# lgalke/aae-recommender

Hardware: AMD Instinct MI355X
Metric: train docs/sec at |items|=100k h=200 (higher is better)
Workload: dtype f32; 1 GPU; C3 PubMed-scale synthetic Bags: |items|=100000, hidden=200, code=50, fp32, batch=100 docs/GPU/step, full partial_fit (ae+disc+gen, 4 Adam) inside the AdversarialAutoEncoder.fit epoch loop (permutation batches of a corpus resident in HBM); n_items=100000, n_hidden=200, n_code=50, batch_per_gpu=100, global_batch=100, cond_inc=0, rng=device, parallelism=dp1

## Files before the change

### aae-recommender_amd/csrc/aae_abi.hip

```cpp
#include <hip/hip_runtime.h>
#include <hip/hip_ext.h>
#include <math.h>
#include <stdio.h>
#include <stdlib.h>
#include <string.h>

#include <algorithm>
#include <string>
#include <vector>

#include "../../include/aaerec_hip.h"
#include "gemm_f32.h"
#include "kernels.h"
#include "dec_fused.h"
#include "dec_fused_bf16.h"
#include "dec_crit_x3.h"
#include "rank_x3.h"
#include "rank_long.h"
#include "rank_full.h"
#include "cooc.h"
#include "spgemm.h"
#include "sptrans.h"
#include "mutinfo.h"
#include "popular.h"
// ... 106 lines not shown
        }
        m->x16_ok = m->use_chain4 && m->FXi[P_W2] != nullptr;
        if (m->x16_ok) each_chain16x3(limit(m->x16_ok, kX16Lds));
        m->force_unfused = cfg->unfused_decoder == 1;
        if (m->fused_ok) {
            each_dec_fused(kDecFused, limit(m->fused_ok, maxlds));
            if (m->bf16) each_dec_fused_bf16(kDecFused, limit(m->fused_ok, maxlds));
            if (!raise_lds_limit(tile_bucket_kernel, maxlds - 2048)) m->fused_ok = false;
            m->bucket_wide_ok = raise_lds_limit(tile_bucket_wide_kernel, maxlds - 16384);
            {
                hipFuncAttributes fa;
                static bool told = false;
                if (m->bucket_wide_ok && !told && hipFuncGetAttributes(&fa, reinterpret_cast<const void*>(tile_bucket_wide_kernel)) == hipSuccess && fa.numRegs < 121) {
                    told = true;
                    fprintf(stderr, "aaerec: tile_bucket_wide_kernel allocates %d vector registers, not the 128 it claims to keep its CU to itself (buckets.h)\n", fa.numRegs);
                }
                (void)hipGetLastError();
            }
        }
    }
    m->late_enabled = !m->opt.no_late_join;
    m->early_enabled = true;
    m->early_any = m->opt.early_any;
    m->rank_ok = m->fused_ok && m->use_chain4 && !m->vae && !m->opt.no_rank_fused;
    m->vae_rank_ok = m->vae && m->fused_ok && m->use_chain4 && !m->opt.no_rank_fused;
    if (m->vae_rank_ok) each_chain4_vae(limit(m->vae_rank_ok, kCSlots * kCR * kCL * sizeof(float)));
    bool& rank_ok = m->vae ? m->vae_rank_ok : m->rank_ok;
    if (rank_ok) each_rank_x3([&](RankKernel k, int nb) { rank_ok = rank_ok && raise_lds_limit(k, rank_x3_lds_bytes(nb)); });
    if (rank_ok) each_rank_x3v2([&](RankKernel k, int nb) { rank_ok = rank_ok && raise_lds_limit(k, rank_x3v2_lds_bytes(nb)); });
    m->w1_big_lds = raise_lds_limit(w1_item_update_kernel, sizeof(int) * w1_items_lds_words(16384));
    (void)hipGetLastError();
    m->grad_scale = 1.f;
    m->rng_row0 = 0; m->rng_global = 0;
    m->Gt = m->G.p;
    m->split_ok = false; m->opt_pending = false; m->side = nullptr; m->ev_crit = m->ev_opt = nullptr;
    m->split_wgs = std::max(1, (m->n_cu * 5) / 8);
    m->pf_armed = m->pf_built = m->pf_pending = false; m->pf_step = -1; m->hstep = 0; m->flushed_hstep = -1; m->ev_head = m->ev_pf = nullptr;
    bool side_ok = false;
    if (cfg->grad_mode == AAE_GRAD_FUSED) {
        int lo = 0, hi = 0;
        const unsigned evflags = hipEventDisableTiming | hipEventDisableSystemFence;
        side_ok = hipDeviceGetStreamPriorityRange(&lo, &hi) == hipSuccess &&
                  hipStreamCreateWithPriority(&m->side, hipStreamNonBlocking, lo) == hipSuccess &&
                  hipEventCreateWithFlags(&m->ev_crit, evflags) == hipSuccess &&
                  hipEventCreateWithFlags(&m->ev_opt, evflags) == hipSuccess &&
                  hipEventCreateWithFlags(&m->ev_head, evflags) == hipSuccess &&
                  hipEventCreateWithFlags(&m->ev_pf, evflags) == hipSuccess &&
                  hipEventCreateWithFlags(&m->ev_bk, evflags) == hipSuccess &&
                  hipEventCreateWithFlags(&m->ev_end, evflags) == hipSuccess;
        if (!side_ok) {
            if (m->side) (void)hipStreamDestroy(m->side);
            m->side = nullptr;
        }
        (void)hipGetLastError();
    }
    if (side_ok && m->fused_ok && m->bf16 && m->split_wgs > 0 &&
        (size_t)((m->N + kBU - 1) / kBU) * kBU * bf_stride(4) <= (size_t)m->R * m->ldn) {
        m->split_ok = true;
        for (int mode : {kDecCrit, kDecOpt}) each_dec_fused_bf16(mode, limit(m->split_ok, maxlds));
        (void)hipGetLastError();
    }
    if (side_ok && m->fused_ok && m->split_wgs > 0 && 
        (size_t)((m->N + kTI - 1) / kTI) * kTI * (size_t)std::min(m->R, 16 * kMB) * sizeof(float) < (size_t)0x7FFFFFF0u) {
        bool ok = true;
        for (int mode : {kDecCrit, kDecOpt, kDecOptAcc}) each_dec_fused(mode, limit(ok, maxlds));
        each_dec_opt_blocks(limit(ok, maxlds));
        if (!m->bf16) m->split_ok = ok;
        m->x3_ok = ok;
        each_dec_crit_x3(false, limit(m->x3_ok, maxlds));
        each_dec_opt_blocks_x3(limit(m->x3_ok, maxlds));
        each_dec_opt_x3(false, limit(m->x3_ok, maxlds));
        (void)hipGetLastError();
        if (m->bf16) {
            m->bf16_x3 = m->x3_ok && ok;
            if (!m->bf16_x3) m->x3_ok = false;
            else m->split_ok = true;
            m->bf16_one = m->bf16_x3;
            each_dec_crit_x3(true, limit(m->bf16_one, maxlds));
            each_dec_opt_x3(true, limit(m->bf16_one, maxlds));
            (void)hipGetLastError();
        }
        if (m->x3_ok) {
            const int ntiles = (m->N + 31) / 32;
            const double t_tile = (3.3 + 0.0131 * m->h) * (m->bf16_one ? 0.87 : 1.0);
            int w = (int)(ntiles * t_tile / (m->bf16_one ? 165.0 : 82.0) / 8.0 + 0.5) * 8;
            w = std::max(w, std::min(ntiles, m->bf16_one ? 48 : 64));
            const int cap = m->late_enabled ? m->n_cu * 15 / 32 : m->n_cu * 9 / 16;
            m->split_wgs = std::max(1, std::min(w, cap));
        }
    }
    hipStream_t s = S(stream);
    hipError_t e = hipMemsetAsync(arena_dev, 0, need, s);
    if (e != hipSuccess) { delete m; return fail(AAE_EHIP, std::string("hipMemsetAsync: ") + hipGetErrorString(e)); }
    struct { Ten* t; int col; } ones[] = {{&m->eh1, m->h}, {&m->eh2, m->h}, {&m->zc, m->cp}, {&m->dh1, m->h},
                                           {&m->dh2, m->h}, {&m->zin, m->c}, {&m->xh1, m->h}, {&m->xh2, m->h}};
    for (auto& o : ones)
        hipLaunchKernelGGL(fill_col_kernel, dim3(((int)o.t->rows + 255) / 256), dim3(256), 0, s, o.t->p, (int)o.t->ld,
                           (int)o.t->rows, o.col, 1.0f);
    OptScalars hs[4]; memset(hs, 0, sizeof(hs));
    for (int i = 0; i < 4; ++i) {
        hs[i].t = 0; hs[i].is_sgd = cfg->optimizer == AAE_OPT_SGD;
        hs[i].lr = (i == O_ENC || i == O_DEC) ? (double)cfg->gen_lr : (double)cfg->reg_lr;
        hs[i].neg_step_size = 0.f; hs[i].bc2_sqrt = 1.f; hs[i].inv_bc2_sqrt = 1.f;
    }
    e = hipMemcpyAsync(m->sc, hs, sizeof(hs), hipMemcpyHostToDevice, s);
    if (e == hipSuccess) e = hipStreamSynchronize(s);
    if (e != hipSuccess) { delete m; return fail(AAE_EHIP, std::string("init: ") + hipGetErrorString(e)); }
    *out = m;
    return AAE_OK;
}

#ifdef W1_TS
int aae_debug_w1_ts(unsigned long long* out, int n) {
    return (int)hipMemcpyFromSymbol(out, HIP_SYMBOL(aae::w1_ts), sizeof(unsigned long long) * (size_t)n);
}
#endif
int aae_destroy(aae_handle h) {
    if (!h) return AAE_OK;
    if (h->side) {
        (void)hipStreamSynchronize(h->side);
        (void)hipStreamDestroy(h->side);
    }
    if (h->dp_scratch) (void)hipFree(h->dp_scratch);
    if (h->cnt_host) (void)hipHostFree(h->cnt_host);
    for (hipEvent_t e : {h->ev_crit, h->ev_opt, h->ev_head, h->ev_pf, h->ev_bk, h->ev_end}) if (e) (void)hipEventDestroy(e);
    if (h->prof_ev) {
        for (int k = 0; k < AAE_K_N; ++k)
            for (auto& pr : h->prof_ev[k]) { (void)hipEventDestroy(pr.first); (void)hipEventDestroy(pr.second); }
        delete[] h->prof_ev;
    }
    delete h;
    return AAE_OK;
}


int aae_profile_enable(aae_handle h, int on) {
    if (!h) return fail(AAE_EINVAL, "handle is NULL");
    if (on && !h->prof_ev) h->prof_ev = new std::vector<std::pair<hipEvent_t, hipEvent_t>>[AAE_K_N];
    h->prof_on = on != 0;
    h->prof_mask = on == 1 ? ~0u : ((unsigned)on >> 1);
    return AAE_OK;
}

int aae_profile_read(aae_handle h, int kernel_id, double* total_ms, int64_t* launches) {
    if (!h || !total_ms || !launches) return fail(AAE_EINVAL, "NULL argument");
    if (kernel_id < 0 || kernel_id >= AAE_K_N) return fail(AAE_EINVAL, "bad kernel id");
    *total_ms = 0.0; *launches = 0;
    if (!h->prof_ev) return AAE_OK;
    auto& v = h->prof_ev[kernel_id];
    for (size_t i = 0; i < h->prof_used[kernel_id]; ++i) {
        HIPCHK(hipEventSynchronize(v[i].second));
        float ms = 0.f;
        HIPCHK(hipEventElapsedTime(&ms, v[i].first, v[i].second));
        *total_ms += ms; *launches += 1;
    }
    h->prof_used[kernel_id] = 0;
    return AAE_OK;
}

int aae_prefetch_batch(aae_handle h, const aae_batch* next) {
    if (!h || !next) return fail(AAE_EINVAL, "NULL argument");
    if (!next->indptr_dev || !next->indices_dev || !next->values_dev) return fail(AAE_EINVAL, "batch pointers are NULL");
    if (next->n_rows < 1 || next->n_rows > h->R) return fail(AAE_EINVAL, "batch n_rows outside [1, max_batch]");
    if (next->nnz_bound > h->cfg.max_nnz) return fail(AAE_EINVAL, "batch nnz_bound > max_nnz");
    if (next->generation == 0) { h->pf_armed = false; return AAE_OK; }
    h->pf_batch = *next;
    h->pf_armed = true;
    return AAE_OK;
}

// ... 117 lines not shown
```

### aae-recommender_amd/csrc/abi_output_layer.h

```cpp
#pragma once

namespace {

struct DecLaunch {
    DecFusedArgs fa;
    int nblk, Bb;
    int ntiles, grid;
    bool win;
    size_t fused_lds;
    bool want_ts, ts_obk;
};
unsigned long long* dec_ts_dev = nullptr;

DecFusedArgs fill_dec_args(const aae_model* m, int B, int nblk, float gscale) {
    DecFusedArgs fa;
    fa.dh2 = m->dh2.p; fa.ldh = m->ldh;
    fa.V3a = m->P[P_V3].p; fa.M = m->M[0][P_V3].p; fa.V = m->V[0][P_V3].p; fa.ldv = m->ldh;
    fa.gradV3 = m->cfg.grad_mode == AAE_GRAD_EXPORT ? m->Gr[P_V3].p : nullptr;
    fa.N = m->N; fa.B = B; fa.h = m->h; fa.gscale = gscale;
    fa.te.start = m->tstart; fa.te.eb = m->teb; fa.te.en = m->ten; fa.te.ev = m->tev;
    fa.slabs = m->slabs.p; fa.slab_stride = (size_t)(nblk > 1 ? B : std::min(m->R, 16 * kMB)) * m->ldh; fa.ld_slab = m->ldh;
    fa.partials = m->bce_partials; fa.sc = m->sc + O_DEC;
    fa.erow0 = 0; fa.acc = nullptr; fa.nblk = 1; fa.Bb = B;
    fa.one_term = m->bf16_x3 ? 1 : 0; fa.dbg_skip = m->opt.dec_skip;
// ... 37 lines not shown
        for (int k = 0; k < 5; ++k) {
            fprintf(stderr, "[dec_fused_bf16 arrivals at barrier %d, us after the unit's start]", k);
            for (int w = 0; w < 16; ++w) fprintf(stderr, " %.2f", ((double)t[16 + 16 * k + w] - (double)t[0]) * 0.01);
            fprintf(stderr, "\n");
        }
    fprintf(stderr, "[dec_fused tile 5] S0=%.2f GEMM1+BCE0=%.2f entries=%.2f GEMM2+GEMM3=%.2f S5=%.2f | tile=%.2f us, %.0f shader clocks -> %.2f GHz\n",
            (t[1] - t[0]) * 0.01, (t[2] - t[1]) * 0.01, (t[3] - t[2]) * 0.01, (t[4] - t[3]) * 0.01,
            (t[6] - t[4]) * 0.01, (t[6] - t[0]) * 0.01, (double)(t[9] - t[8]),
            (double)(t[9] - t[8]) / ((t[6] - t[0]) * 10.0));
    if (out_bf16(m)) fprintf(stderr, "[dec_fused_bf16 S0] barrier A=%.2f work=%.2f barrier B=%.2f us\n", (t[14] - t[0]) * 0.01, (t[15] - t[14]) * 0.01, (t[1] - t[15]) * 0.01);
    fprintf(stderr, "[dec_fused wg 0] prologue=%.2f loop=%.2f (%llu tiles, %.2f each) epilogue=%.2f us\n",
            (t[11] - t[10]) * 0.01, (t[7] - t[11]) * 0.01, t[13], (t[7] - t[11]) * 0.01 / (double)(t[13] ? t[13] : 1),
            (t[12] - t[7]) * 0.01);
    return AAE_OK;
}

int launch_output_critical(aae_model* m, const DecLaunch& L, bool late, int grid, hipStream_t s) {
    DecFusedArgs b = L.fa;
    b.nblk = L.nblk; b.Bb = L.Bb;
    if (late) { b.dh2_snap = m->dh2s.p; b.sc_snap = m->sc_snap; }
    hipEvent_t start = nullptr, stop = m->ev_crit;
    (void)prof_pair(m, AAE_K_DEC_CRIT, &start, &stop);
    const int nb = m->fused_nb;
    DecKernel kernel; int threads = kNT; uint32_t lds = (uint32_t)L.fused_lds;
    if (out_bf16(m)) { kernel = pick_dec_fused_bf16(nb, kDecCrit); threads = kBT; }
    else if (m->x3_ok) {
        const bool ts = b.ts && !m->bf16_one && nb == 13;
        kernel = pick_dec_crit_x3(nb, ts, m->bf16_one, L.win && !ts);
        lds = (uint32_t)dec_crit_x3_lds_bytes(nb);
    } else kernel = pick_dec_fused(nb, kDecCrit, L.win);
    if (!kernel) return no_kernel("dec_fused (critical launch)");
    hipExtLaunchKernelGGL(kernel, dim3(grid), dim3(threads), lds, s, start, stop, 0, b);
    LAUNCHCHK("dec_fused (critical launch)");
    HIPCHK(hipStreamWaitEvent(m->side, stop, 0));
    return AAE_OK;
}

int launch_deferred(aae_model* m, DecKernel kernel, const char* what, int grid, int threads, uint32_t lds, const DecFusedArgs& b) {
    if (!kernel) return no_kernel(what);
    hipEvent_t start = nullptr, stop = nullptr;
    (void)prof_pair(m, AAE_K_DEC_OPT, &start, &stop);
    hipExtLaunchKernelGGL(kernel, dim3(grid), dim3(threads), lds, m->side, start, stop, 0, b);
    LAUNCHCHK(what);
    return AAE_OK;
}

int launch_output_deferred(aae_model* m, const DecLaunch& L, bool late, bool* late_launched) {
    const DecFusedArgs& fa = L.fa;
    const int nblk = L.nblk, Bb = L.Bb, ntiles = L.ntiles, nb = m->fused_nb, B = fa.B;
    const int g2 = std::min(ntiles, std::min(m->split_wgs, m->n_cu));
    DecFusedArgs b = fa;
    b.nblk = nblk; b.Bb = Bb;
    if (nblk > 1 && !out_bf16(m) && m->x3_ok && m->dh2f.p) {
        hipLaunchKernelGGL(dh2_frag_kernel, dim3((B + kXCH - 1) / kXCH, m->fused_nb), dim3(128), 0, m->side, m->dh2.p, m->ldh, B,
                           reinterpret_cast<u32x4_t*>(m->dh2f.p), b.one_term);
        b.acc = m->dh2f.p;
        const int wg_cap = ntiles >= 4096 ? m->n_cu * 7 / 8 : m->n_cu * 3 / 4;
        const int by_tiles = ntiles < 384 ? std::max(32, std::min(m->n_cu / 2, ntiles / 3))
                                          : std::max(m->n_cu / 2, std::min(wg_cap, (int)(ntiles / 16.3 / 8.0 + 0.5) * 8));
        const int g3 = std::max(1, std::min(by_tiles, std::min(ntiles, m->n_cu)));
        const int rounds = (ntiles + g3 * kXBT - 1) / (g3 * kXBT);
        b.tpp = g3 * rounds;
        const uint32_t lds3 = (uint32_t)dec_opt_blocks_x3_lds_bytes();
        const bool ts = L.ts_obk && nb == 13;
        TRY(launch_deferred(m, pick_dec_opt_blocks_x3(nb, ts, L.win && !ts), "dec_opt_blocks_x3", g3, kNT, lds3, b));
        return ts ? print_dec_timeline(m, true, false, m->side) : AAE_OK;
    }
    if (nblk > 1 && !out_bf16(m) && ntiles <= kOBT * m->n_cu && dec_opt_blocks_lds_bytes(Bb) <= 160 * 1024) {
        const int g3 = std::max(std::min(g2, ntiles), (ntiles + kOBT - 1) / kOBT);
        return launch_deferred(m, pick_dec_opt_blocks(nb), "dec_opt_blocks", g3, kNT, (uint32_t)dec_opt_blocks_lds_bytes(Bb), b);
    }
    for (int r = 0; r < nblk; ++r) {
        b = fa;
        const int r0 = r * Bb;
        b.B = std::min(Bb, B - r0); b.erow0 = r0;
        b.dh2 = fa.dh2 + (size_t)r0 * m->ldh;
        b.slabs = fa.slabs + (size_t)r0 * m->ldh;
        b.partials = fa.partials + (size_t)r * L.grid;
        b.Gt = fa.Gt + (size_t)r * ntiles * Bb * kTI;
        if (nblk > 1) { b.acc = m->Gacc.p; b.gradV3 = r == nblk - 1 ? nullptr : m->Gacc.p; }
        const char* what = "dec_fused (optimiser launch)";
        if (out_bf16(m)) TRY(launch_deferred(m, pick_dec_fused_bf16(nb, kDecOpt), what, g2, kBT, (uint32_t)L.fused_lds, b));
        else if (nblk == 1 && m->x3_ok) {
            const uint32_t lds_nat = (uint32_t)dec_opt_x3_lds_bytes();
            const uint32_t lds3 = m->bf16_one ? std::max(lds_nat, 150u * 1024u) : lds_nat;
            if (late) { b.dh2 = m->dh2s.p; b.sc = m->sc_snap; *late_launched = true; }
            TRY(launch_deferred(m, pick_dec_opt_x3(nb, m->bf16_one, L.win), what, g2, kNT, lds3, b));
        } else TRY(launch_deferred(m, pick_dec_fused(nb, r == 0 ? kDecOpt : kDecOptAcc, L.win), what, g2, kNT, (uint32_t)L.fused_lds, b));
    }
    return AAE_OK;
}

int output_layer_split(aae_model* m, const DecLaunch& L, int* n_loss_partials, int* crit_slabs, hipStream_t s) {
    if (m->opt_pending) TRY(join_deferred(m, s));
    const int nblk = L.nblk;
    const bool late = m->late_enabled && nblk == 1 && m->x3_ok && !out_bf16(m) && !L.want_ts &&
                      m->dh2s.p && m->sc_snap && L.fa.B <= m->dh2s.rows && L.grid >= L.fa.B;
    const int wgs = nblk > 1 ? std::max(1, m->n_cu / nblk) : L.grid;
    const int crit_grid = nblk > 1 ? wgs * nblk : L.grid;
    *n_loss_partials = crit_grid;
    *crit_slabs = wgs;
    TRY(launch_output_critical(m, L, late, crit_grid, s));
    bool late_launched = false;
    TRY(launch_output_deferred(m, L, late, &late_launched));
    TRY(side_done(m, m->ev_opt));
    m->opt_pending = true;
    m->late_ok = late_launched;
    m->last_out_split = true; m->side_ordered = true;
    if (m->only_output_layer && m->pf_armed && m->mark2 && m->lazy) TRY(launch_prefetch(m, false));
    return AAE_OK;
}

int launch_output_single(aae_model* m, const DecLaunch& L, hipStream_t s) {
    m->last_out_split = false; m->side_ordered = false;
    ProfScope ps(m, AAE_K_DEC_FUSED, s);
    const DecKernel kernel = m->bf16 ? pick_dec_fused_bf16(m->fused_nb, kDecFused) : pick_dec_fused(m->fused_nb, kDecFused, L.win);
    if (!kernel) return no_kernel("dec_fused");
    const size_t lds = m->bf16 ? dec_fused_bf16_lds_bytes(m->fused_nb) : L.fused_lds;
    hipLaunchKernelGGL(kernel, dim3(L.grid), dim3(m->bf16 ? kBT : kNT), lds, s, L.fa);
    return AAE_OK;
}

int reduce_slabs(aae_model* m, const DecLaunch& L, int crit_slabs, int n_loss_partials, const DropSpec& d2, const float** part_out, hipStream_t s) {
    const int B = L.fa.B, N = m->N, h = m->h;
    const size_t slab_stride = L.fa.slab_stride;
    float* part = m->slabs.p + (size_t)304 * slab_stride;
    *part_out = part;
    const size_t n4 = (size_t)B * m->ldh / 4;
    auto sum_slabs = [&](const float* src, int n, float* dst, size_t dst_stride, int ny, bool loss) {
        hipLaunchKernelGGL(slab_partial_kernel, dim3((unsigned)((n4 + 255) / 256), ny), dim3(256), 0, s, src, n, slab_stride, n4, dst, dst_stride,
                           loss ? m->bce_partials : (const float*)nullptr, loss ? n_loss_partials : 0, loss ? 1.0f / ((float)B * (float)N) : 0.f, m->losses, 0);
    };
    if (m->only_output_layer && crit_slabs <= 64) {
        sum_slabs(m->slabs.p, crit_slabs, m->da2.p, 0, 1, true);
        LAUNCHCHK("slabs -> da2");
        return AAE_OK;
    }
    sum_slabs(m->slabs.p, crit_slabs, part, slab_stride, 16, true);
    if (m->only_output_layer) {
        sum_slabs(part, 16, m->da2.p, 0, 1, false);
        LAUNCHCHK("slab_partial -> da2");
    } else if (!m->use_chain) {
        hipLaunchKernelGGL(slab_reduce_actbwd_kernel, dim3(grid1d((size_t)B * h, 64)), dim3(64), 0, s, part, 16,
                           slab_stride, B, h, m->ldh, m->dh2.p, m->ldh, m->gb0.p, m->cfg.activation, d2,
                           m->cfg.seed, m->step_ctr);
        LAUNCHCHK("slab_reduce");
    }
    return AAE_OK;
}

int output_layer_fused(aae_model* m, int B, float gscale, const DropSpec& d2, const float** chain_part, size_t* chain_stride, hipStream_t s) {
    if (m->bk_pending) {
        HIPCHK(hipStreamWaitEvent(s, m->ev_bk, 0));
        m->bk_pending = false;
    }
    if (!m->buckets_valid) TRY(build_tile_buckets(m, s));
    DecLaunch L;
    L.nblk = m->have_batch ? row_blocks(m) : 1; L.Bb = (B + L.nblk - 1) / L.nblk;
    L.ntiles = (m->N + kTI - 1) / kTI; L.grid = std::min(L.ntiles, m->n_cu);
    L.win = x3_big_span(m->N, m->ldh);
    L.fused_lds = out_bf16(m) ? dec_fused_bf16_lds_bytes(m->fused_nb) : dec_fused_lds_bytes(L.Bb, m->h);
    L.fa = fill_dec_args(m, B, L.nblk, gscale);
    L.want_ts = m->opt.dec_ts[0] != 0;
    if (L.want_ts) {
        if (!dec_ts_dev && hipMalloc(&dec_ts_dev, 128 * sizeof(unsigned long long)) != hipSuccess) return fail(AAE_EHIP, "ts alloc");
        L.fa.ts = dec_ts_dev;
    }
// ... 144 lines not shown
```

### aae-recommender_amd/csrc/dec_crit_x3.h

```cpp
#pragma once
#include "dec_fused_bf16.h"

namespace aae {

typedef short s16x4_t __attribute__((ext_vector_type(4)));

__device__ __forceinline__ void split3_pair(float a, float b, unsigned& p1, unsigned& p2, unsigned& p3, bool one) {
    x3_split_pair(a, b, p1, p2, p3);
    if (one) { p2 = 0u; p3 = 0u; }
}
__device__ __forceinline__ f32x4 mfma_x3(const bf16x8 (&a)[3], const bf16x8 (&b)[3], f32x4 c) { return x3_mfma(a, b, c); }
template <bool ONE>
__device__ __forceinline__ f32x4 mfma_xt(const bf16x8 (&a)[3], const bf16x8 (&b)[3], f32x4 c) {
    if constexpr (ONE) return __builtin_amdgcn_mfma_f32_16x16x32_bf16(a[0], b[0], c, 0, 0, 0);
    else return x3_mfma(a, b, c);
}

__host__ __device__ constexpr int x3_stride(int kc) { return 16 * kc + 8; }
__device__ __forceinline__ bf16x8 x3_frag(const unsigned* img, int row, int S, int kc, int fk) {
    return __builtin_bit_cast(bf16x8, *reinterpret_cast<const u32x4_t*>(img + row * S + 16 * kc + 4 * fk));
}
constexpr int kXRS = 33;
constexpr int kXT = 32;

// ... 285 lines not shown
            const int lz = lane + oz, q = (lz >> 2) & 3, p = lz & 3;
            const unsigned* base = v3K + (8 * fkz + q) * S1 + 8 * cb + 2 * p;
#pragma unroll
            for (int t = 0; t < NT; ++t) {
                const s16x4_t lo = __builtin_amdgcn_ds_read_tr16_b64_v4i16(
                    (s16x4_t __attribute__((address_space(3)))*)(base + t * (kTI * S1)));
                const s16x4_t hi = __builtin_amdgcn_ds_read_tr16_b64_v4i16(
                    (s16x4_t __attribute__((address_space(3)))*)(base + t * (kTI * S1) + 4 * S1));
                typedef short s16x8_t __attribute__((ext_vector_type(8)));
                const s16x8_t v = {lo[0], lo[1], lo[2], lo[3], hi[0], hi[1], hi[2], hi[3]};
                vt[t] = __builtin_bit_cast(bf16x8, v);
            }
        };
        auto gemm3 = [&](auto Q0, auto Q1) {
#pragma unroll
            for (int q = decltype(Q0)::value; q < decltype(Q1)::value; ++q) {
                if (BAL && (q < q_lo || q >= q_hi)) continue;
                bf16x8 ga[3];
#pragma unroll
                for (int t = 0; t < NT; ++t) ga[t] = x3_frag(gK + t * (kGR * S3), 16 * q + frz, S3, 0, fkz);
                acc3[q] = mfma_xt<ONE>(ga, vt, acc3[q]);
            }
        };
        typedef std::integral_constant<int, 0> Q_0;
        typedef std::integral_constant<int, kMB> Q_E;
        constexpr int NJ = (kGR * (kTI / 2) + kNT - 1) / kNT;
        stamp(0);

        stamp(14);
        stamp(1);
        if (kCritG1Pf) {
            if (g1) { if (nks == NKS) gemm1_pf(std::integral_constant<int, NKS>()); else gemm1_pf(std::integral_constant<int, (NKS > 1 ? NKS - 1 : 1)>()); }
        } else if (g1) gemm1();
        load_span(min(tile + stride, ntiles - 1), vreg);
        lds_barrier();
        stamp(2);
        lprod = 1.f;
#pragma unroll
        for (int j = 0; j < NJ; ++j) bce(64 * wave + kNT * j);
        loss += log_pos(lprod);
        if (own) read_vt();
        lds_barrier();
        stamp(3);
        if (own) gemm3(Q_0(), Q_E());
        __builtin_amdgcn_sched_barrier(0);
        stage(tile + stride);
        stamp(4);
        __builtin_amdgcn_sched_barrier(0);
        lds_barrier();
        __builtin_amdgcn_sched_barrier(0);
        stamp(5);
        stamp(6);
    }
    if (TS && a.ts && blockIdx.x == 0 && tid == 0) a.ts[7] = wall_clock64();

    float* slab = slabs_blk + (size_t)wgi * a.slab_stride;
    if (own) {
#pragma unroll
        for (int q = 0; q < kMB; ++q) {
            const int rb = q * 16 + fk * 4, cc = cb * 16 + fr;
#pragma unroll
            for (int r = 0; r < 4; ++r)
                if (q >= q_lo && q < q_hi && rb + r < B && cc < a.ld_slab) slab[(size_t)(rb + r) * a.ld_slab + cc] = acc3[q][r];
        }
    }
    loss = wave_sum(loss);
    __syncthreads();
    if (lane == 0) red[wave] = loss;
    __syncthreads();
    if (tid == 0) {
        float s = 0.f;
        for (int w = 0; w < kNW; ++w) s += red[w];
        a.partials[blockIdx.x] = s;
        if (TS && a.ts && blockIdx.x == 0) { a.ts[12] = wall_clock64(); a.ts[13] = (unsigned long long)iter; }
    }
}

}

namespace aae {

constexpr int kXGS = 20;

inline size_t dec_opt_x3_lds_bytes() { return sizeof(float) * ((size_t)3 * 128 * kXGS + (size_t)kTI * kSO + 64); }

template <int NB, bool ONE = false, bool WIN = false>
__global__ __launch_bounds__(kNT) void dec_opt_x3_kernel(DecFusedArgs a) {
    const bool one = ONE || a.one_term != 0;
    constexpr int NT = ONE ? 1 : 3;
    constexpr int KR = 4;
    static_assert(NB <= 13, "column blocks 10..12 are the ones split over two waves");
    extern __shared__ __attribute__((aligned(16))) float lds[];
    unsigned* gB = reinterpret_cast<unsigned*>(lds);
    float* os = reinterpret_cast<float*>(gB + 3 * 128 * kXGS);
    const int tid = threadIdx.x, lane = tid & 63;
    const int wave = __builtin_amdgcn_readfirstlane(tid >> 6);
    const int fr = lane & 15, fk = lane >> 4;
    const int B = a.B, ldv = a.ldv, N = a.N;
    const int ntiles = (N + kTI - 1) / kTI;
    const int f4_per_row = ldv / 4, tile_f4 = kTI * f4_per_row;
    constexpr int NV = 2;
    const OptScalars sc = *a.sc;
    const bool do_adam = a.gradV3 == nullptr;
    typedef unsigned int fu32x4 __attribute__((ext_vector_type(4)));
    if (a.dbg_skip & 0x10000) return;
    if (a.dbg_skip & 0x20000) {
        const unsigned long long t0 = wall_clock64();
        while (wall_clock64() - t0 < 13500ull) __builtin_amdgcn_s_sleep(32);
        return;
    }

    for (int i = tid; i < 3 * 128 * kXGS; i += kNT) gB[i] = 0u;

    int cb, nb_lo, nb_hi;
    if (wave < 10) { cb = wave; nb_lo = 0; nb_hi = 2; }
    else { cb = 10 + ((wave - 10) >> 1); nb_lo = (wave - 10) & 1; nb_hi = nb_lo + 1; }
    const bool live = cb < NB;
    cb = min(cb, NB - 1);
    bf16x8 dB[KR][3];
    {
        const int c = min(16 * cb + fr, a.ldh - 1);
#pragma unroll
        for (int kc = 0; kc < KR; ++kc) {
            float x[8];
#pragma unroll
            for (int j = 0; j < 8; ++j) {
                const int b = 32 * kc + 8 * fk + j;
                x[j] = (b < B && 16 * cb + fr < a.ldh) ? a.dh2[(size_t)b * a.ldh + c] : 0.f;
            }
            unsigned p[3][4];
#pragma unroll
            for (int q = 0; q < 4; ++q) split3_pair(x[2 * q], x[2 * q + 1], p[0][q], p[1][q], p[2][q], one);
#pragma unroll
            for (int t = 0; t < NT; ++t) {
                const u32x4_t v = {p[t][0], p[t][1], p[t][2], p[t][3]};
                dB[kc][t] = __builtin_bit_cast(bf16x8, v);
            }
        }
    }

    const unsigned lane_off = (unsigned)tid * 16u;
    const unsigned tile_bytes = (unsigned)(kTI * ldv) * 4u;
    X3WindowT<WIN> win(N, ldv, tile_bytes);
    const float* gbase = a.gradV3 ? a.gradV3 : a.V3a;
    __amdgpu_buffer_rsrc_t rP = win.desc(a.V3a), rM = win.desc(a.M), rV = win.desc(a.V), rG = win.desc(gbase);
    const int g_f4 = B * (kTI / 4);
    const unsigned gbytes = (unsigned)min((size_t)0x7FFFFFF0u, (size_t)ntiles * g_f4 * 16);
    const __amdgpu_buffer_rsrc_t rGt = __builtin_amdgcn_make_buffer_rsrc(a.Gt, 0, gbytes, 0x00020000);
    auto ld4 = [&](const __amdgpu_buffer_rsrc_t& r, int tile, int j) {
        const unsigned vo = tid + kNT * j < tile_f4 ? lane_off + (unsigned)(kNT * 16 * j) : 0x80000000u;
        return __builtin_bit_cast(float4, __builtin_amdgcn_raw_buffer_load_b128(r, vo, win.so(tile), 2));
    };
    auto ldg = [&](int tile) {
        return __builtin_bit_cast(float4, __builtin_amdgcn_raw_buffer_load_b128(rGt, tid < g_f4 ? lane_off : 0x80000000u, (unsigned)tile * (unsigned)g_f4 * 16u, 2));
    };
    int s_rc[NV];
#pragma unroll
    for (int j = 0; j < NV; ++j) {
        const int fc = min(tid + kNT * j, tile_f4 - 1), row = fc / f4_per_row;
        s_rc[j] = row * 64 + (fc - row * f4_per_row);
    }
    float4 p_cur[NV], p_nxt[NV], mreg[NV], sreg[NV], g_nxt;
    int tile = blockIdx.x;
    const int stride = gridDim.x;
    if (tile < ntiles) {
#pragma unroll
        for (int j = 0; j < NV; ++j) p_nxt[j] = ld4(rP, tile, j);
        g_nxt = ldg(tile);
    }
    __syncthreads();

    for (; tile < ntiles; tile += stride) {
        const int i0 = tile * kTI;
        if (win.moves(tile)) { rP = win.desc(a.V3a); rM = win.desc(a.M); rV = win.desc(a.V); rG = win.desc(gbase); }
        int oz;
        asm volatile("v_mov_b32 %0, 0" : "=v"(oz));
        const int lz = lane + oz;
        lds_barrier();
        if (tid < g_f4) {
            unsigned q0[3], q1[3];
            split3_pair(g_nxt.x, g_nxt.y, q0[0], q0[1], q0[2], one);
            split3_pair(g_nxt.z, g_nxt.w, q1[0], q1[1], q1[2], one);
            unsigned* d = gB + (tid >> 3) * kXGS + (tid & 7) * 2;
#pragma unroll
            for (int t = 0; t < NT; ++t) *reinterpret_cast<uint2*>(d + t * (128 * kXGS)) = make_uint2(q0[t], q1[t]);
        }
#pragma unroll
        for (int j = 0; j < NV; ++j) p_cur[j] = p_nxt[j];
        g_nxt = ldg(min(tile + stride, ntiles - 1));
#pragma unroll
        for (int j = 0; j < NV; ++j) p_nxt[j] = ld4(rP, min(tile + stride, ntiles - 1), j);
#pragma unroll
        for (int j = 0; j < NV; ++j) { mreg[j] = ld4(rM, tile, j); sreg[j] = ld4(rV, tile, j); }
        lds_barrier();

        if (live) {
            const int tq = (lz >> 2) & 3, tp = lz & 3, g = lz >> 4;
            for (int nb2 = nb_lo; nb2 < nb_hi; ++nb2) {
                f32x4 c = (f32x4){0.f, 0.f, 0.f, 0.f};
                const unsigned* base = gB + (8 * g + tq) * kXGS + 8 * nb2 + 2 * tp;
#pragma unroll
                for (int kc = 0; kc < KR; ++kc) {
                    bf16x8 ga[3];
#pragma unroll
                    for (int t = 0; t < NT; ++t) {
                        const unsigned* pb = base + t * (128 * kXGS) + 32 * kc * kXGS;
                        const s16x4_t lo = __builtin_amdgcn_ds_read_tr16_b64_v4i16((s16x4_t __attribute__((address_space(3)))*)(pb));
                        const s16x4_t hi = __builtin_amdgcn_ds_read_tr16_b64_v4i16((s16x4_t __attribute__((address_space(3)))*)(pb + 4 * kXGS));
                        typedef short s16x8_t __attribute__((ext_vector_type(8)));
                        const s16x8_t v = {lo[0], lo[1], lo[2], lo[3], hi[0], hi[1], hi[2], hi[3]};
                        ga[t] = __builtin_bit_cast(bf16x8, v);
                    }
                    c = mfma_xt<ONE>(ga, dB[kc], c);
                }
#pragma unroll
                for (int r = 0; r < 4; ++r) os[(16 * nb2 + 4 * fk + r) * kSO + 16 * cb + fr] = c[r];
            }
        }
        lds_barrier();

#pragma unroll
        for (int j = 0; j < NV; ++j) {
            const bool valid = tid + kNT * j < tile_f4 && i0 + (s_rc[j] >> 6) < N;
            const float4 g = *reinterpret_cast<const float4*>(os + (s_rc[j] >> 6) * kSO + (s_rc[j] & 63) * 4);
            const unsigned so = win.so(tile);
            const unsigned vo = valid ? lane_off + (unsigned)(kNT * 16 * j) : 0x80000000u;
            float4 p = p_cur[j], mm = mreg[j], vv = sreg[j];
            adam_update(p.x, mm.x, vv.x, g.x, sc); adam_update(p.y, mm.y, vv.y, g.y, sc);
            adam_update(p.z, mm.z, vv.z, g.z, sc); adam_update(p.w, mm.w, vv.w, g.w, sc);
            const float4 out = do_adam ? p : g;
            const unsigned vo2 = (do_adam && !sc.is_sgd) ? vo : 0x80000000u;
            __builtin_amdgcn_raw_buffer_store_b128(__builtin_bit_cast(fu32x4, out), do_adam ? rP : rG, vo, so, 2);
            __builtin_amdgcn_raw_buffer_store_b128(__builtin_bit_cast(fu32x4, mm), rM, vo2, so, 2);
            __builtin_amdgcn_raw_buffer_store_b128(__builtin_bit_cast(fu32x4, vv), rV, vo2, so, 2);
        }
    }
}


constexpr int kXBT = 6;
constexpr int kXCH = 64;
constexpr int kXRowTab = 768;
constexpr int kXRing = 6;

__device__ __forceinline__ void glds16(const void* gsrc, unsigned lds_dst) {
    unsigned keep;
    asm volatile("s_mov_b32 %0, m0\n\ts_mov_b32 m0, %2\n\ts_nop 0\n\tglobal_load_lds_dwordx4 %1, off nt\n\ts_mov_b32 m0, %0"
                 : "=&s"(keep) : "v"(gsrc), "s"(lds_dst) : "memory");
}

inline size_t dec_opt_blocks_x3_lds_bytes() { return sizeof(float) * std::max((size_t)2 * 3 * 2 * kXCH * 8 + (size_t)kXRing * kXCH * kTI + 256 + 9 * kXRowTab, (size_t)kXBT * kTI * kSO); }

__global__ __launch_bounds__(128) void dh2_frag_kernel(const float* __restrict__ dh2, int ldh, int B, u32x4_t* __restrict__ out, int one_term) {
    const bool one = one_term != 0;
    const int ch = blockIdx.x, cb = blockIdx.y, nb = gridDim.y;
    const int kc = threadIdx.x >> 6, lane = threadIdx.x & 63, fr = lane & 15, fk = lane >> 4;
    const int c = 16 * cb + fr;
    float x[8];
#pragma unroll
    for (int j = 0; j < 8; ++j) {
        const int b = kXCH * ch + 32 * kc + 8 * fk + j;
        x[j] = (b < B && c < ldh) ? dh2[(size_t)b * ldh + c] : 0.f;
    }
    unsigned p[3][4];
#pragma unroll
    for (int q = 0; q < 4; ++q) split3_pair(x[2 * q], x[2 * q + 1], p[0][q], p[1][q], p[2][q], one);
#pragma unroll
    for (int t = 0; t < 3; ++t) {
        const u32x4_t v = {p[t][0], p[t][1], p[t][2], p[t][3]};
        out[((((size_t)ch * nb + cb) * (kXCH / 32) + kc) * 3 + t) * 64 + lane] = v;
    }
}

template <int NB, bool TS = false, bool WIN = false>
__global__ __launch_bounds__(kNT) void dec_opt_blocks_x3_kernel(DecFusedArgs a) {
    const bool one = a.one_term != 0;
    constexpr int KR = kXCH / 32;
    constexpr int IMG = 2 * kXCH * 8;
    auto slot_of = [](int r) { return (r & ~12) | ((r & 4) << 1) | ((r & 8) >> 1); };
    static_assert(NB <= kNW, "one column block per wave");
    extern __shared__ __attribute__((aligned(16))) float lds[];
    unsigned* gB = reinterpret_cast<unsigned*>(lds);
    float* ring = lds + 2 * 3 * IMG;
    unsigned* rowtab = reinterpret_cast<unsigned*>(ring + kXRing * kXCH * kTI + 256);
    float* os = lds;
    const int tid = threadIdx.x, lane = tid & 63;
    const int wave = __builtin_amdgcn_readfirstlane(tid >> 6);
    const int fr = lane & 15, fk = lane >> 4;
    const int ldv = a.ldv, N = a.N, B = a.B;
    const int ntiles = (N + kTI - 1) / kTI;
    const int f4_per_row = ldv / 4, tile_f4 = kTI * f4_per_row;
    constexpr int NV = 2;
    const OptScalars sc = *a.sc;
    typedef unsigned int fu32x4 __attribute__((ext_vector_type(4)));
    const int G = max(a.tpp, 1);
    const int nch = (B + kXCH - 1) / kXCH;
    const int cb = min(wave, NB - 1);

    const unsigned lane_off = (unsigned)tid * 16u;
    const unsigned tile_bytes = (unsigned)(kTI * ldv) * 4u;
    X3WindowT<WIN> win(N, ldv, tile_bytes);
    __amdgpu_buffer_rsrc_t rP = win.desc(a.V3a), rM = win.desc(a.M), rV = win.desc(a.V);
    auto ld4 = [&](const __amdgpu_buffer_rsrc_t& r, int tile, int j) {
        return __builtin_bit_cast(float4, __builtin_amdgcn_raw_buffer_load_b128(r, lane_off + (unsigned)(kNT * 16 * j), win.so(tile), 2));
    };
    constexpr int NM = NB + 1;
    constexpr int NL = (kNW - NM) * 64, NS = (kXCH * 8 + NL - 1) / NL;
    static_assert(NM < kNW, "no spare wave left");
    static_assert(kXCH * 8 * 2 == kNT, "one float4 of a slot per thread of the lower half");
    const bool mult = wave < NM;
    const int nb_lo = wave == NB ? 1 : 0, nb_hi = wave == NB - 1 ? 1 : 2;
    const int lt = tid - NM * 64;
// ... 197 lines not shown
```

Before: 432,600 docs/s.

## Prefetch next tile's Adam state interleaved with MFMA steps in dec_opt_x3

The x3 decoder optimiser kernel now prefetches the next tile's M and V moments along with P and the gradient. The individual prefetch loads are spread across the MFMA k-steps with scheduling barriers, so memory latency overlaps the GEMM instead of stalling before it. The third bf16 term of the decoder fragments moves from registers to LDS to reduce register pressure, and the Adam update is inlined with hardcoded beta constants. The split-workgroup heuristic constants are also retuned. Risks: more LDS per block, and the inlined update assumes beta1=0.9 and beta2=0.999.

After: 438,500 docs/s (median of 6 runs). 1.01x the previous value.

```diff
diff --git a/aae-recommender_amd/csrc/aae_abi.hip b/aae-recommender_amd/csrc/aae_abi.hip
--- a/aae-recommender_amd/csrc/aae_abi.hip
+++ b/aae-recommender_amd/csrc/aae_abi.hip
@@ -212,10 +212,10 @@
         }
         if (m->x3_ok) {
             const int ntiles = (m->N + 31) / 32;
-            const double t_tile = (3.3 + 0.0131 * m->h) * (m->bf16_one ? 0.87 : 1.0);
-            int w = (int)(ntiles * t_tile / (m->bf16_one ? 165.0 : 82.0) / 8.0 + 0.5) * 8;
-            w = std::max(w, std::min(ntiles, m->bf16_one ? 48 : 64));
-            const int cap = m->late_enabled ? m->n_cu * 15 / 32 : m->n_cu * 9 / 16;
+            const double t_tile = (2.2 + 0.0096 * m->h) * (m->bf16_one ? 0.98 : 1.0);
+            int w = (int)(ntiles * t_tile / (m->bf16_one ? 127.0 : 57.0) / 8.0 + 0.5) * 8;
+            w = std::max(w, std::min(ntiles, m->bf16_one ? 40 : 64));
+            const int cap = m->late_enabled ? m->n_cu * 7 / 16 : m->n_cu * 9 / 16;
             m->split_wgs = std::max(1, std::min(w, cap));
         }
     }
diff --git a/aae-recommender_amd/csrc/abi_output_layer.h b/aae-recommender_amd/csrc/abi_output_layer.h
--- a/aae-recommender_amd/csrc/abi_output_layer.h
+++ b/aae-recommender_amd/csrc/abi_output_layer.h
@@ -143,7 +143,7 @@
         const char* what = "dec_fused (optimiser launch)";
         if (out_bf16(m)) TRY(launch_deferred(m, pick_dec_fused_bf16(nb, kDecOpt), what, g2, kBT, (uint32_t)L.fused_lds, b));
         else if (nblk == 1 && m->x3_ok) {
-            const uint32_t lds_nat = (uint32_t)dec_opt_x3_lds_bytes();
+            const uint32_t lds_nat = (uint32_t)dec_opt_x3_lds_bytes(!m->bf16_one);
             const uint32_t lds3 = m->bf16_one ? std::max(lds_nat, 150u * 1024u) : lds_nat;
             if (late) { b.dh2 = m->dh2s.p; b.sc = m->sc_snap; *late_launched = true; }
             TRY(launch_deferred(m, pick_dec_opt_x3(nb, m->bf16_one, L.win), what, g2, kNT, lds3, b));
diff --git a/aae-recommender_amd/csrc/dec_crit_x3.h b/aae-recommender_amd/csrc/dec_crit_x3.h
--- a/aae-recommender_amd/csrc/dec_crit_x3.h
+++ b/aae-recommender_amd/csrc/dec_crit_x3.h
@@ -391,7 +391,13 @@
 
 constexpr int kXGS = 20;
 
-inline size_t dec_opt_x3_lds_bytes() { return sizeof(float) * ((size_t)3 * 128 * kXGS + (size_t)kTI * kSO + 64); }
+constexpr int kXDL = 16 * 4 * 64;
+
+inline size_t dec_opt_x3_lds_bytes(bool three_term) {
+    const size_t base = sizeof(float) * ((size_t)3 * 128 * kXGS + (size_t)kTI * kSO + 64);
+    static_assert((3 * 128 * kXGS + kTI * kSO + 64) % 4 == 0, "the third-term block is read 16 bytes at a time");
+    return base + (three_term ? (size_t)kXDL * 16 : 0);
+}
 
 template <int NB, bool ONE = false, bool WIN = false>
 __global__ __launch_bounds__(kNT) void dec_opt_x3_kernel(DecFusedArgs a) {
@@ -402,6 +408,7 @@
     extern __shared__ __attribute__((aligned(16))) float lds[];
     unsigned* gB = reinterpret_cast<unsigned*>(lds);
     float* os = reinterpret_cast<float*>(gB + 3 * 128 * kXGS);
+    u32x4_t* dB2 = reinterpret_cast<u32x4_t*>(os + kTI * kSO + 64);
     const int tid = threadIdx.x, lane = tid & 63;
     const int wave = __builtin_amdgcn_readfirstlane(tid >> 6);
     const int fr = lane & 15, fk = lane >> 4;
@@ -426,7 +433,9 @@
     else { cb = 10 + ((wave - 10) >> 1); nb_lo = (wave - 10) & 1; nb_hi = nb_lo + 1; }
     const bool live = cb < NB;
     cb = min(cb, NB - 1);
-    bf16x8 dB[KR][3];
+    constexpr int NR = ONE ? 1 : 2;
+    bf16x8 dB[KR][NR];
+    u32x4_t* const dB2w = dB2 + (wave * KR) * 64 + lane;
     {
         const int c = min(16 * cb + fr, a.ldh - 1);
 #pragma unroll
@@ -443,7 +452,8 @@
 #pragma unroll
             for (int t = 0; t < NT; ++t) {
                 const u32x4_t v = {p[t][0], p[t][1], p[t][2], p[t][3]};
-                dB[kc][t] = __builtin_bit_cast(bf16x8, v);
+                if (t < NR) dB[kc][t] = __builtin_bit_cast(bf16x8, v);
+                else dB2w[kc * 64] = v;
             }
         }
     }
@@ -456,12 +466,12 @@
     const int g_f4 = B * (kTI / 4);
     const unsigned gbytes = (unsigned)min((size_t)0x7FFFFFF0u, (size_t)ntiles * g_f4 * 16);
     const __amdgpu_buffer_rsrc_t rGt = __builtin_amdgcn_make_buffer_rsrc(a.Gt, 0, gbytes, 0x00020000);
-    auto ld4 = [&](const __amdgpu_buffer_rsrc_t& r, int tile, int j) {
-        const unsigned vo = tid + kNT * j < tile_f4 ? lane_off + (unsigned)(kNT * 16 * j) : 0x80000000u;
+    auto ld4 = [&](const __amdgpu_buffer_rsrc_t& r, int tile, bool there, int j) {
+        const unsigned vo = there && tid + kNT * j < tile_f4 ? lane_off + (unsigned)(kNT * 16 * j) : 0x80000000u;
         return __builtin_bit_cast(float4, __builtin_amdgcn_raw_buffer_load_b128(r, vo, win.so(tile), 2));
     };
-    auto ldg = [&](int tile) {
-        return __builtin_bit_cast(float4, __builtin_amdgcn_raw_buffer_load_b128(rGt, tid < g_f4 ? lane_off : 0x80000000u, (unsigned)tile * (unsigned)g_f4 * 16u, 2));
+    auto ldg = [&](int tile, bool there) {
+        return __builtin_bit_cast(float4, __builtin_amdgcn_raw_buffer_load_b128(rGt, there && tid < g_f4 ? lane_off : 0x80000000u, (unsigned)tile * (unsigned)g_f4 * 16u, 2));
     };
     int s_rc[NV];
 #pragma unroll
@@ -469,13 +479,22 @@
         const int fc = min(tid + kNT * j, tile_f4 - 1), row = fc / f4_per_row;
         s_rc[j] = row * 64 + (fc - row * f4_per_row);
     }
-    float4 p_cur[NV], p_nxt[NV], mreg[NV], sreg[NV], g_nxt;
+    float4 p_cur[NV], p_nxt[NV], m_cur[NV], m_nxt[NV], s_cur[NV], s_nxt[NV], g_nxt;
+    auto upd = [&](float& p, float& m, float& v, float g) {
+        if (sc.is_sgd) { p = __builtin_fmaf(sc.neg_step_size, g, p); return; }
+        m = __builtin_fmaf(0.1f, g - m, m);
+        v = __builtin_fmaf(0.001f * g, g, v * 0.999f);
+        const float denom = __builtin_fmaf(__builtin_amdgcn_sqrtf(v), sc.inv_bc2_sqrt, 1e-8f);
+        p = __builtin_fmaf(sc.neg_step_size * m, __builtin_amdgcn_rcpf(denom), p);
+    };
     int tile = blockIdx.x;
     const int stride = gridDim.x;
     if (tile < ntiles) {
-#pragma unroll
-        for (int j = 0; j < NV; ++j) p_nxt[j] = ld4(rP, tile, j);
-        g_nxt = ldg(tile);
+        g_nxt = ldg(tile, true);
+#pragma unroll
+        for (int j = 0; j < NV; ++j) p_nxt[j] = ld4(rP, tile, true, j);
+#pragma unroll
+        for (int j = 0; j < NV; ++j) { m_nxt[j] = ld4(rM, tile, true, j); s_nxt[j] = ld4(rV, tile, true, j); }
     }
     __syncthreads();
 
@@ -495,21 +514,30 @@
             for (int t = 0; t < NT; ++t) *reinterpret_cast<uint2*>(d + t * (128 * kXGS)) = make_uint2(q0[t], q1[t]);
         }
 #pragma unroll
-        for (int j = 0; j < NV; ++j) p_cur[j] = p_nxt[j];
-        g_nxt = ldg(min(tile + stride, ntiles - 1));
-#pragma unroll
-        for (int j = 0; j < NV; ++j) p_nxt[j] = ld4(rP, min(tile + stride, ntiles - 1), j);
-#pragma unroll
-        for (int j = 0; j < NV; ++j) { mreg[j] = ld4(rM, tile, j); sreg[j] = ld4(rV, tile, j); }
-        lds_barrier();
-
-        if (live) {
-            const int tq = (lz >> 2) & 3, tp = lz & 3, g = lz >> 4;
-            for (int nb2 = nb_lo; nb2 < nb_hi; ++nb2) {
-                f32x4 c = (f32x4){0.f, 0.f, 0.f, 0.f};
-                const unsigned* base = gB + (8 * g + tq) * kXGS + 8 * nb2 + 2 * tp;
-#pragma unroll
-                for (int kc = 0; kc < KR; ++kc) {
+        for (int j = 0; j < NV; ++j) { p_cur[j] = p_nxt[j]; m_cur[j] = m_nxt[j]; s_cur[j] = s_nxt[j]; }
+        lds_barrier();
+
+        const bool there = tile + stride < ntiles;
+        const int tn = min(tile + stride, ntiles - 1);
+        auto req = [&](auto I) {
+            constexpr int i = decltype(I)::value, j = (i - 1) / 3, w = (i - 1) % 3;
+            if constexpr (i == 0) g_nxt = ldg(tn, there);
+            else if constexpr (w == 0) p_nxt[j] = ld4(rP, tn, there, j);
+            else if constexpr (w == 1) m_nxt[j] = ld4(rM, tn, there, j);
+            else s_nxt[j] = ld4(rV, tn, there, j);
+        };
+
+        const int tq = (lz >> 2) & 3, tp = lz & 3, gq = lz >> 4;
+        auto gemm2 = [&](auto IT) {
+            constexpr int it = decltype(IT)::value;
+            const bool act = live && nb_lo + it < nb_hi;
+            const int nb2 = nb_lo + it;
+            f32x4 c = (f32x4){0.f, 0.f, 0.f, 0.f};
+            const unsigned* base = gB + (8 * gq + tq) * kXGS + 8 * nb2 + 2 * tp;
+            auto kstep = [&](auto KC) {
+                constexpr int kc = decltype(KC)::value;
+                if constexpr (4 * it + kc < 7) req(std::integral_constant<int, (4 * it + kc < 7 ? 4 * it + kc : 0)>());
+                if (act) {
                     bf16x8 ga[3];
 #pragma unroll
                     for (int t = 0; t < NT; ++t) {
@@ -520,12 +548,22 @@
                         const s16x8_t v = {lo[0], lo[1], lo[2], lo[3], hi[0], hi[1], hi[2], hi[3]};
                         ga[t] = __builtin_bit_cast(bf16x8, v);
                     }
-                    c = mfma_xt<ONE>(ga, dB[kc], c);
-                }
+                    bf16x8 db[3];
+#pragma unroll
+                    for (int t = 0; t < NT; ++t) db[t] = t < NR ? dB[kc][t < NR ? t : 0] : __builtin_bit_cast(bf16x8, dB2w[kc * 64 + oz]);
+                    c = mfma_xt<ONE>(ga, db, c);
+                }
+                __builtin_amdgcn_sched_barrier(0);
+            };
+            kstep(std::integral_constant<int, 0>()); kstep(std::integral_constant<int, 1>());
+            kstep(std::integral_constant<int, 2>()); kstep(std::integral_constant<int, 3>());
+            if (act) {
 #pragma unroll
                 for (int r = 0; r < 4; ++r) os[(16 * nb2 + 4 * fk + r) * kSO + 16 * cb + fr] = c[r];
             }
-        }
+        };
+        gemm2(std::integral_constant<int, 0>());
+        gemm2(std::integral_constant<int, 1>());
         lds_barrier();
 
 #pragma unroll
@@ -534,9 +572,9 @@
             const float4 g = *reinterpret_cast<const float4*>(os + (s_rc[j] >> 6) * kSO + (s_rc[j] & 63) * 4);
             const unsigned so = win.so(tile);
             const unsigned vo = valid ? lane_off + (unsigned)(kNT * 16 * j) : 0x80000000u;
-            float4 p = p_cur[j], mm = mreg[j], vv = sreg[j];
-            adam_update(p.x, mm.x, vv.x, g.x, sc); adam_update(p.y, mm.y, vv.y, g.y, sc);
-            adam_update(p.z, mm.z, vv.z, g.z, sc); adam_update(p.w, mm.w, vv.w, g.w, sc);
+            float4 p = p_cur[j], mm = m_cur[j], vv = s_cur[j];
+            upd(p.x, mm.x, vv.x, g.x); upd(p.y, mm.y, vv.y, g.y);
+            upd(p.z, mm.z, vv.z, g.z); upd(p.w, mm.w, vv.w, g.w);
             const float4 out = do_adam ? p : g;
             const unsigned vo2 = (do_adam && !sc.is_sgd) ? vo : 0x80000000u;
             __builtin_amdgcn_raw_buffer_store_b128(__builtin_bit_cast(fu32x4, out), do_adam ? rP : rG, vo, so, 2);
```
